# GMC-DRL/MetaBox

Measured on AMD Instinct MI355X. Metric: env-steps/sec (instances x gens/s), RLEPSO bbob-easy d=10, higher is better.
Workload: dtype f64

## Files before the change

### metabox_amd/csrc/mbx_device.hpp

```cpp
#pragma once
#include <type_traits>
#include <hip/hip_runtime.h>
#include <stdint.h>

#include "../../include/mbx.h"
#include "../../include/mbx_layout.h"
#include "mbx_math.hpp"

namespace mbx {

#ifdef MBX_NOINLINE_MATH
#define MBX_MATH __device__ __noinline__
#else
#define MBX_MATH __device__ __forceinline__
#endif
#ifdef MBX_LIBM_MATH
MBX_MATH double m_pow(double a, double b) { return pow(a, b); }
MBX_MATH double m_sin(double a) { return sin(a); }
MBX_MATH double m_cos(double a) { return cos(a); }
MBX_MATH double m_exp(double a) { return exp(a); }
MBX_MATH double m_log(double a) { return log(a); }
#else
MBX_MATH double m_pow(double a, double b) { return fm::pow_fast(a, b); }
MBX_MATH double m_sin(double a) { return fm::sincos_fast<false>(a); }
MBX_MATH double m_cos(double a) { return fm::sincos_fast<true>(a); }
MBX_MATH double m_exp(double a) { return fm::exp_fast(a); }
MBX_MATH double m_log(double a) { return fm::log_fast(a); }
#endif


constexpr int kThreads = 256;
#define MBX_NT ((int)blockDim.x)
#define MBX_NW ((int)blockDim.x >> 6)
constexpr double kTwoPi = 6.283185307179586;

struct DevProblem {
    int32_t func_id, kind, dim, n_peaks, noise_kind;
    int32_t n_close;
    double bias, lb, ub, pen_coef, s[4], noise_a, noise_b, optimum;
    const double *dshift, *m1, *m2, *v0, *v1, *v2, *py, *pc, *pw;
    const double* pyr;
    const double* plogw;
};

typedef const DevProblem __attribute__((address_space(4))) ConstProblem;

struct FastDiv {
    uint32_t m, one; int D;
    __device__ __forceinline__ explicit FastDiv(int D_) : m(0xFFFFFFFFu / (uint32_t)D_ + 1u), one(D_ == 1 ? 0xFFFFFFFFu : 0u), D(D_) {}
    __device__ __forceinline__ int div(int e) const { return (int)(__umulhi((uint32_t)e, m) + ((uint32_t)e & one)); }
    __device__ __forceinline__ int mod(int e) const { return e - div(e) * D; }
};

struct U4 { uint32_t x, y, z, w; };

__device__ __forceinline__ U4 philox4x32_10(uint32_t c0, uint32_t c1, uint32_t c2, uint32_t c3, uint32_t k0, uint32_t k1)
{
#ifndef MBX_PHILOX_ROUNDS
#define MBX_PHILOX_ROUNDS 10
#endif
#pragma unroll
    for (int r = 0; r < MBX_PHILOX_ROUNDS; ++r) {
        const uint64_t p0 = (uint64_t)MBX_PHILOX_M0 * c0, p1 = (uint64_t)MBX_PHILOX_M1 * c2;
        const uint32_t hi0 = (uint32_t)(p0 >> 32), lo0 = (uint32_t)p0;
        const uint32_t hi1 = (uint32_t)(p1 >> 32), lo1 = (uint32_t)p1;
#ifdef MBX_PHILOX_XOR2
        const uint32_t n0 = hi1 ^ c1 ^ k0, n2 = hi0 ^ c3 ^ k1;
#else
        const uint32_t n0 = __builtin_amdgcn_bitop3_b32(hi1, c1, k0, 0x96), n2 = __builtin_amdgcn_bitop3_b32(hi0, c3, k1, 0x96);
#endif
        c0 = n0; c1 = lo1; c2 = n2; c3 = lo0;
        k0 += MBX_PHILOX_W0; k1 += MBX_PHILOX_W1;
    }
    return U4{c0, c1, c2, c3};
}

__device__ __forceinline__ double u53(uint32_t a, uint32_t b)
{
    return ((double)(a >> 5) * 67108864.0 + (double)(b >> 6)) * (1.0 / 9007199254740992.0);
}

__device__ __forceinline__ double u32d(uint32_t a) { return (double)a * 2.3283064365386963e-10; }

struct Rng {
    uint32_t k0, k1, gen, episode;
    bool uniform_fresh = false;
    __device__ __forceinline__ U4 draw(uint32_t idx, uint32_t site) const
    {
#ifdef MBX_ABLATE_RNG
        return U4{idx * 2654435761u, site + 0x9E3779B9u * idx, gen ^ (idx << 7), episode + idx};
#else
        uint32_t a = k0, b = k1;
        if (uniform_fresh) {
            a = (uint32_t)__builtin_amdgcn_readfirstlane((int)a); b = (uint32_t)__builtin_amdgcn_readfirstlane((int)b);
            asm volatile("" : "+s"(a), "+s"(b));
        }
        return philox4x32_10(idx, site, gen, episode, a, b);
#endif
    }
};

__device__ __forceinline__ void box_muller(double ua, double ub, double& n0, double& n1)
{
    const double r = sqrt(-2.0 * m_log(1.0 - ua));
    const double t = kTwoPi * ub;
    n0 = r * m_cos(t);
    n1 = r * m_sin(t);
}

__device__ __forceinline__ void philox_noise(const Rng& rng, uint32_t row, uint32_t siteA, uint32_t siteB, int noise_kind,
                                             double& a, double& b, double& c)
{
    a = b = c = 0.0;
    if (noise_kind == MBX_NOISE_NONE) return;
    U4 w = rng.draw(row, siteA);
    const double ua = u53(w.x, w.y), ub = u53(w.z, w.w);
    if (noise_kind == MBX_NOISE_GAUSS) {
        a = sqrt(-2.0 * m_log(1.0 - ua)) * m_cos(kTwoPi * ub);
    } else if (noise_kind == MBX_NOISE_UNIFORM) {
        a = ua; b = ub;
    } else {
        a = ua;
        w = rng.draw(row, siteB);
        box_muller(u53(w.x, w.y), u53(w.z, w.w), b, c);
    }
}

template <class PT>
__device__ __forceinline__ double apply_noise(const PT& P, double ftrue, double a, double b, double c)
{
    if (P.noise_kind == MBX_NOISE_NONE) return ftrue;
    const double fu = ftrue - P.optimum;
    double fn;
    if (P.noise_kind == MBX_NOISE_GAUSS) {
        fn = fu * m_exp(P.noise_a * a);
    } else if (P.noise_kind == MBX_NOISE_UNIFORM) {
        fn = fu * m_pow(a, P.noise_b) * fmax(1., m_pow(1e9 / (fu + 1e-99), P.noise_a * (0.49 + 1. / P.dim) * b));
    } else {
        fn = fu + P.noise_a * fmax(0., 1e3 + (a < P.noise_b ? 1. : 0.) * b / (fabs(c) + 1e-199));
    }
    return fu >= 1e-8 ? fn + P.optimum + 1.01 * 1e-8 : ftrue;
}

__device__ __forceinline__ int opaque_tid()
{
    int t = (int)threadIdx.x;
    asm volatile("" : "+v"(t));
    return t;
}

__device__ __forceinline__ void wave_argmin(double& v, int& i)
{
#pragma unroll
    for (int off = 32; off >= 1; off >>= 1) {
        const double ov = __shfl_xor(v, off, 64);
        const int oi = __shfl_xor(i, off, 64);
        if (ov < v || (ov == v && oi < i)) { v = ov; i = oi; }
    }
}

__device__ __forceinline__ void block_argmin(const double* a, int n, double* red, double& vmin, int& imin)
{
    const int tid = opaque_tid();
    if (tid < 64) {
        double v = INFINITY; int idx = 0x7fffffff;
        for (int j = tid; j < n; j += 64) {
            const double x = a[j];
            if (x < v) { v = x; idx = j; }
        }
        wave_argmin(v, idx);
        if (idx >= n) { idx = 0; v = a[0]; }
        if (tid == 0) { red[0] = v; red[1] = (double)idx; }
    }
    __syncthreads();
    vmin = red[0]; imin = (int)red[1];
    __syncthreads();
}


__device__ __forceinline__ double div_by_tenth(double L)
{
    const double q = L * 10.0;
    return __builtin_fma(__builtin_fma(-0.1, q, L), 10.0, q);
}

__device__ __forceinline__ double osc1(double x)
{
    if (x == 0.) return x;
    const bool pos = x > 0.;
    const double y = div_by_tenth(m_log(fabs(x)));
    const double c1 = pos ? 1.0 : 0.55, c2 = pos ? 0.79 : 0.31;
    const double r = m_exp(0.1 * (y + 0.49 * (m_sin(c1 * y) + m_sin(c2 * y))));
    return pos ? r : -r;
}

#if defined(MBX_NOINLINE_MATH) && !defined(MBX_LIBM_MATH)
__device__ __noinline__ double osc1_composite(double x)
{
    if (x == 0.) return x;
    const bool pos = x > 0.;
    const double y = div_by_tenth(fm::log_fast(fabs(x)));
    const double c1 = pos ? 1.0 : 0.55, c2 = pos ? 0.79 : 0.31;
    const double r = fm::exp_fast(0.1 * (y + 0.49 * (fm::sincos_fast<false>(c1 * y) + fm::sincos_fast<false>(c2 * y))));
    return pos ? r : -r;
}
__device__ __noinline__ double schaffers_composite(double s)
{
    const double w = fm::sincos_fast<false>(50 * fm::pow_fast(s, 0.2));
    return sqrt(s) * (w * w + 1);
}
#else
__device__ __forceinline__ double osc1_composite(double x) { return osc1(x); }
__device__ __forceinline__ double schaffers_composite(double s) { return sqrt(s) * (m_pow(m_sin(50 * m_pow(s, 0.2)), 2) + 1); }
#endif
#ifndef MBX_COMPOSITE_DC
#define MBX_COMPOSITE_DC 10
#endif
template <bool CMP> __device__ __forceinline__ double osc_t(double x) { if constexpr (CMP) return osc1_composite(x); else return osc1(x); }

__device__ __forceinline__ double asy1(double x, double beta_lin)
{
    return x > 0. ? m_pow(x, 1. + beta_lin * sqrt(x)) : x;
}

__device__ __forceinline__ double pen_row(const double* x, int D, double ub)
{
    double s = 0.;
    for (int d = 0; d < D; ++d) {
        const double t = fmax(0., fabs(x[d]) - ub);
        s += t * t;
    }
    return s;
}

__host__ __device__ inline long long eval_t_doubles(int n, int D)
{
    long long t = (long long)n * D;
    if (t < 17ll * D) t = 17ll * D;
    if (t < 8ll * n) t = 8ll * n;
    return (t + 1) & ~1ll;
}

struct EvalLds {
    const double* X;
// ... 843 lines not shown
```

### metabox_amd/csrc/mbx_rlepso.hpp

```cpp
#pragma once
#include "mbx_device.hpp"

namespace mbx {

struct BatchParams {
    const DevProblem* problems;
    const int32_t* problem_idx;
    const uint64_t* seeds;
    double* state;
    int64_t state_stride;
    const double* tape;
    int64_t tape_stride;
    const int32_t* order;
    const double* pci;
    int32_t NP, D, max_fes, log_interval, n_logpoint, early_stop, n_group, B;
    int64_t sc_off;
    unsigned long long* clk;
};

template <class PT>
__device__ __forceinline__ bool log_and_terminate(const BatchParams& bp, const PT& P, double fes, double gbest, int& log_index,
                                                  int& cost_len, double* __restrict__ cost)
{
    if (fes >= (double)log_index * bp.log_interval) { log_index += 1; cost[cost_len++] = gbest; }
// ... 67 lines not shown
    L.DSH = p; p += align2(D);
    L.V0 = p; p += align2(D);
    L.V1 = p; p += align2(D);
    L.V2 = p; p += align2(D);
    L.PBC = p; p += P;
    L.NC = p; p += P;
    L.PNI = p; p += P;
    L.CMUT = p; p += P;
    L.GB = p; p += align2(D);
    L.RED = p; p += 16;
    L.IMPR = (int*)p; p += align2((P + 1) / 2);
    L.MASK = (int*)p; p += align2((P + 1) / 2);
    L.RANK = (int*)p;
    return L;
}

__device__ __forceinline__ void rl_commit(const RlLds& L, int NP, int D, bool stagnation, double& gbest, int& gbest_idx,
                                          double* __restrict__ gPB, double* __restrict__ gCC)
{
    const int tid = threadIdx.x;
    for (int i = tid; i < NP; i += MBX_NT) {
        const double nc = L.NC[i];
        if (stagnation) L.PNI[i] = nc < gCC[i] ? 0. : L.PNI[i] + 1;
        const int impr = nc < L.PBC[i];
        if (impr) L.PBC[i] = nc;
        L.IMPR[i] = impr;
        gCC[i] = nc;
    }
    double cbv; int cb;
    block_argmin(L.NC, NP, L.RED, cbv, cb);
    const bool better = cbv < gbest;
    if (better) { gbest = cbv; gbest_idx = cb; }
    const int NE = NP * D;
    const FastDiv fd(D);
    for (int e = tid; e < NE; e += MBX_NT) {
        const int i = fd.div(e);
        if (L.IMPR[i]) gPB[e] = L.X[e];
    }
    if (better && tid < D) L.GB[tid] = L.X[cb * D + tid];
    __syncthreads();
}

struct MoveCtx {
    const RlLds& L; const double* pci; const double* tape; const Rng& rng; double* gPos; double* gVel;
    const int* ORDER; const int* NLESS; const int* RANK; int NP, D, G; double lb, ub, vmax; const FastDiv& fg;
};

struct GaussMlp {
    const float* w;
    int32_t in_dim, h1, h2, out_dim;
    float min_sigma, max_sigma;
    int32_t variant;
};

__host__ __device__ inline int gauss_mlp_net_floats(int in, int h1, int h2, int A) { return in * h1 + h1 + h1 * h2 + h2 + h2 * A + A; }

__device__ __forceinline__ void gauss_head(const GaussMlp& net, float am, float as, float& mu, float& sigma)
{
    mu = (tanhf(am) + 1.f) / 2.f;
    if (net.variant == MBX_POLICY_RLPSO) sigma = fminf(fmaxf((tanhf(as) + 1.f) / 2.f, net.min_sigma), net.max_sigma);
    else sigma = (tanhf(as) + 1.f) / 2.f * (net.max_sigma - net.min_sigma) + net.min_sigma;
}

__device__ __forceinline__ float sample_action(const Rng& rng, int j, float mu, float sigma, int variant)
{
    const U4 w = rng.draw((uint32_t)j, MBX_SITE_POLICY);
    const float u1 = (float)((w.x >> 8) + 1u) * 5.9604644775390625e-8f;
    const float u2 = (float)(w.y >> 8) * 5.9604644775390625e-8f;
    const float r = __builtin_sqrtf(-1.3862943611198906f * __builtin_amdgcn_logf(u1));
    const float a = mu + sigma * (r * __builtin_amdgcn_cosf(u2));
    if (variant == MBX_POLICY_RLPSO) return fabsf(a - 0.5f) >= 0.5f ? (a + 3.f * sigma - mu) * ((1.f / 6.f) * sigma) : a;
    return fminf(fmaxf(a, 0.f), 1.f);
}

#ifdef MBX_PHASE_TIMING
__device__ unsigned long long g_phase_cycles[8192 * 16];
#define MBX_PHASE_BEGIN unsigned long long ph_t = clock64();
#define MBX_PHASE(k) do { if (threadIdx.x == 0) { const unsigned long long t_ = clock64(); g_phase_cycles[(blockIdx.x & 8191) * 16 + (k)] += t_ - ph_t; ph_t = t_; } } while (0)
#else
#define MBX_PHASE_BEGIN
#define MBX_PHASE(k)
#endif

#ifndef MBX_RL_WAVES
#define MBX_RL_WAVES __attribute__((amdgpu_waves_per_eu(THREADS == 256 ? 5 : 4)))
#endif
#ifndef MBX_FDR_UNROLL
#define MBX_FDR_UNROLL 4
#endif
#ifndef MBX_FDR_OWN_AT
#define MBX_FDR_OWN_AT 64
#endif

__device__ __forceinline__ void fdr_take(double lhs, double rhs, double& ab, double& bb, int& kb, double a, double b, int k)
{
#ifdef MBX_FDR_BRANCH
    if (__builtin_amdgcn_ballot_w64(lhs < rhs) == 0ull) return;
#endif
#ifdef MBX_FDR_SELECT
    if (lhs < rhs) { ab = a; bb = b; kb = k; }
#else
    unsigned long long saved;
    asm("s_mov_b64 %[sv], exec\n\t"
                 "v_cmpx_lt_f64_e32 %[l], %[r]\n\t"
                 "v_mov_b64 %[ab], %[a]\n\t"
                 "v_mov_b64 %[bb], %[b]\n\t"
                 "v_mov_b32 %[kb], %[k]\n\t"
                 "s_mov_b64 exec, %[sv]"
                 : [ab] "+v"(ab), [bb] "+v"(bb), [kb] "+v"(kb), [sv] "=&s"(saved)
                 : [l] "v"(lhs), [r] "v"(rhs), [a] "v"(a), [b] "v"(b), [k] "s"(k)
                 : "vcc");
#endif
}

__device__ __forceinline__ void fdr_take_neg(double dif, double& ab, double& bb, int& kb, double a, double b, int k)
{
    unsigned long long saved;
    asm("s_mov_b64 %[sv], exec\n\t"
        "v_cmpx_gt_f64_e32 0, %[d]\n\t"
        "v_mov_b64 %[ab], %[a]\n\t"
        "v_mov_b64 %[bb], %[b]\n\t"
        "v_mov_b32 %[kb], %[k]\n\t"
        "s_mov_b64 exec, %[sv]"
        : [ab] "+v"(ab), [bb] "+v"(bb), [kb] "+v"(kb), [sv] "=&s"(saved)
        : [d] "v"(dif), [a] "v"(a), [b] "v"(b), [k] "s"(k)
        : "vcc");
}
__device__ __forceinline__ void fdr_take_neg2(double dif0, double dif1, double& ab0, double& bb0, int& kb0, double& ab1, double& bb1, int& kb1,
                                              double a, double b0, double b1, int k)
{
    unsigned long long saved;
    asm("s_mov_b64 %[sv], exec\n\t"
        "v_cmpx_gt_f64_e32 0, %[d0]\n\t"
        "v_mov_b64 %[ab0], %[a]\n\t"
        "v_mov_b64 %[bb0], %[b0]\n\t"
        "v_mov_b32 %[kb0], %[k]\n\t"
        "s_mov_b64 exec, %[sv]\n\t"
        "v_cmpx_gt_f64_e32 0, %[d1]\n\t"
        "v_mov_b64 %[ab1], %[a]\n\t"
        "v_mov_b64 %[bb1], %[b1]\n\t"
        "v_mov_b32 %[kb1], %[k]\n\t"
        "s_mov_b64 exec, %[sv]"
        : [ab0] "+v"(ab0), [bb0] "+v"(bb0), [kb0] "+v"(kb0), [ab1] "+v"(ab1), [bb1] "+v"(bb1), [kb1] "+v"(kb1), [sv] "=&s"(saved)
        : [d0] "v"(dif0), [d1] "v"(dif1), [a] "v"(a), [b0] "v"(b0), [b1] "v"(b1), [k] "s"(k)
        : "vcc");
}
__device__ __forceinline__ float f64_hi_as_f32(double v) { return __int_as_float(__double2hiint(v)); }
__device__ __forceinline__ float fdr_min3_abs(float m, float x, float y)
{
    float r;
    asm("v_min3_f32 %[r], %[m], |%[x]|, |%[y]|" : [r] "=v"(r) : [m] "v"(m), [x] "v"(x), [y] "v"(y));
    return r;
}
__device__ __forceinline__ void rl_mark_copies(const RlLds& L, int NP, int D, int r)
{
    if (r > 0 && r < NP && L.NC[r] == L.NC[r - 1]) {
        bool same = true;
        for (int d = 0; d < D && same; ++d) same = L.PB[r * D + d] == L.PB[(r - 1) * D + d];
        if (same) L.NCS[r] = 1e300;
    }
}

__device__ __forceinline__ int fdr_settle(const RlLds& L, const int* __restrict__ ORDER, int D, int rk, int d, int nless, int kw, unsigned long long* cnt = nullptr)
{
    const int lane = threadIdx.x & 63;
    const double fi = L.NC[rk];
    const double pp = L.PB[rk * D + d];
    const double aw = L.NC[kw] - fi, bw = fabs(L.PB[kw * D + d] - pp) + 1e-5;
    int first_copy = 0x7fffffff;
    bool others = false;
    for (int k0 = 0; k0 < nless; k0 += 64) {
        const int k = k0 + lane;
        bool band = false, copy = false;
        if (k < nless && k != kw) {
            const double a = L.NC[k] - fi, b = fabs(L.PB[k * D + d] - pp) + 1e-5, pr = aw * b;
            band = __builtin_fma(a, bw, -pr) <= pr * -0x1p-49;
            copy = band && a == aw && b == bw;
        }
        const unsigned long long mc = __builtin_amdgcn_ballot_w64(copy), mo = __builtin_amdgcn_ballot_w64(band && !copy);
        if (mc != 0ull && first_copy == 0x7fffffff) first_copy = k0 + (int)__builtin_ctzll(mc);
        others = others || mo != 0ull;
    }
    int kbest = kw < first_copy ? kw : first_copy;
#ifdef MBX_FDR_COUNT
    if (cnt && lane == 0) atomicAdd(cnt + (others ? 5 : first_copy != 0x7fffffff ? 4 : 6), 1ull);
#endif
    if (others) {
        double qb = aw / bw;
        int ib = ORDER[kbest];
        for (int k0 = 0; k0 < nless; k0 += 64) {
            const int k = k0 + lane;
            bool cont = false;
            double qk = 0.;
            int ik = 0;
            if (k < nless && k != kw) {
                const double a = L.NC[k] - fi, b = fabs(L.PB[k * D + d] - pp) + 1e-5, pr = aw * b;
                cont = __builtin_fma(a, bw, -pr) <= pr * -0x1p-49 && !(a == aw && b == bw);
                if (cont) { qk = a / b; ik = ORDER[k]; }
            }
            unsigned long long m = __builtin_amdgcn_ballot_w64(cont);
            while (m != 0ull) {
                const int l = (int)__builtin_ctzll(m);
                m &= m - 1ull;
                const double ql = __hiloint2double(__builtin_amdgcn_readlane(__double2hiint(qk), l), __builtin_amdgcn_readlane(__double2loint(qk), l));
                const int il = __builtin_amdgcn_readlane(ik, l);
                if (ql < qb || (ql == qb && il < ib)) { qb = ql; ib = il; kbest = k0 + l; }
            }
        }
    }
    return kbest;
}

template <int W, int UN = MBX_FDR_UNROLL, bool TIE = true>
__device__ __forceinline__ bool fdr_exact(const RlLds& L, int D, int rk, int d0, int nless, int kb[W], double range = 0.)
{
#pragma unroll
    for (int q = 0; q < W; ++q) kb[q] = nless;
    if (nless <= 0) return false;
    const double fi = L.NC[rk];
    double pp[W], ab[W], bb[W];
    const double a0 = L.NC[0] - fi;
#pragma unroll
    for (int q = 0; q < W; ++q) { pp[q] = L.PB[rk * D + d0 + q]; kb[q] = 0; ab[q] = a0; bb[q] = fabs(L.PB[d0 + q] - pp[q]) + 1e-5; }
    const double* col = L.PB + d0;
    if constexpr (TIE) {
    float tiem = __int_as_float(0x7f000000);
    auto step = [&](double au, const double (&x)[W], int k) {
        double b[W], difv[W];
#pragma unroll
        for (int q = 0; q < W; ++q) b[q] = fabs(x[q] - pp[q]) + 1e-5;
#pragma unroll
        for (int q = 0; q < W; ++q) difv[q] = ab[q] * b[q];
#pragma unroll
        for (int q = 0; q < W; ++q) difv[q] = __builtin_fma(au, bb[q], -difv[q]);
        if constexpr (W == 2) fdr_take_neg2(difv[0], difv[1], ab[0], bb[0], kb[0], ab[1], bb[1], kb[1], au, b[0], b[1], k);
        else {
#pragma unroll
            for (int q = 0; q < W; ++q) fdr_take_neg(difv[q], ab[q], bb[q], kb[q], au, b[q], k);
        }
        tiem = fdr_min3_abs(tiem, f64_hi_as_f32(difv[0]), f64_hi_as_f32(difv[W - 1]));
    };
    int k = 1;
    for (; k + UN <= nless; k += UN) {
        double a[UN], x[UN][W];
#pragma unroll
        for (int u = 0; u < UN; ++u) {
            a[u] = L.NCS[k + u];
#pragma unroll
            for (int q = 0; q < W; ++q) x[u][q] = col[(k + u) * D + q];
        }
#pragma unroll
        for (int u = 0; u < UN; ++u) step(a[u] - fi, x[u], k + u);
    }
    for (; k < nless; ++k) {
        double x[W];
#pragma unroll
        for (int q = 0; q < W; ++q) x[q] = col[k * D + q];
        step(L.NCS[k] - fi, x, k);
    }
    const double thr = fabs(a0) * range * 0x1p-49;
    return !(tiem > f64_hi_as_f32(thr) * 1.0000005f);
    } else {
    int k = 1;
    for (; k + UN <= nless; k += UN) {
        double a[UN], x[UN][W];
#pragma unroll
        for (int u = 0; u < UN; ++u) {
            a[u] = L.NCS[k + u];
#pragma unroll
            for (int q = 0; q < W; ++q) x[u][q] = col[(k + u) * D + q];
        }
#pragma unroll
        for (int u = 0; u < UN; ++u) {
            const double au = a[u] - fi;
#pragma unroll
            for (int q = 0; q < W; ++q) {
                const double b = fabs(x[u][q] - pp[q]) + 1e-5;
                fdr_take(au * bb[q], ab[q] * b, ab[q], bb[q], kb[q], au, b, k + u);
            }
        }
    }
    for (; k < nless; ++k) {
        const double a = L.NCS[k] - fi;
#pragma unroll
        for (int q = 0; q < W; ++q) {
            const double b = fabs(col[k * D + q] - pp[q]) + 1e-5;
            fdr_take(a * bb[q], ab[q] * b, ab[q], bb[q], kb[q], a, b, k);
        }
    }
    return false;
    }
}

template <int W>
__device__ __noinline__ void fdr_settle_own(const double* __restrict__ NC, const double* __restrict__ PB, const int* __restrict__ ORDER, int D, int rk, int d0, int nless, int* kb)
{
    const double fi = NC[rk];
    double pp[W], aw[W], bw[W];
    int kw[W], first_copy[W];
    bool others[W];
#pragma unroll
    for (int q = 0; q < W; ++q) {
        kw[q] = kb[q];
        pp[q] = PB[rk * D + d0 + q];
        aw[q] = NC[kw[q]] - fi;
        bw[q] = fabs(PB[kw[q] * D + d0 + q] - pp[q]) + 1e-5;
        first_copy[q] = 0x7fffffff; others[q] = false;
    }
    for (int k = 0; k < nless; ++k) {
        const double a = NC[k] - fi;
#pragma unroll
        for (int q = 0; q < W; ++q) {
            const double b = fabs(PB[k * D + d0 + q] - pp[q]) + 1e-5, pr = aw[q] * b;
            if (__builtin_fma(a, bw[q], -pr) <= pr * -0x1p-49 && k != kw[q]) {
                if (a == aw[q] && b == bw[q]) { if (first_copy[q] == 0x7fffffff) first_copy[q] = k; }
                else others[q] = true;
            }
        }
    }
#pragma unroll
    for (int q = 0; q < W; ++q) {
        kb[q] = kw[q] < first_copy[q] ? kw[q] : first_copy[q];
        if (others[q]) {
            double qb = aw[q] / bw[q];
            int ib = ORDER[kb[q]];
            for (int k = 0; k < nless; ++k) {
                const double a = NC[k] - fi, b = fabs(PB[k * D + d0 + q] - pp[q]) + 1e-5, pr = aw[q] * b;
                if (__builtin_fma(a, bw[q], -pr) <= pr * -0x1p-49 && k != kw[q] && !(a == aw[q] && b == bw[q])) {
                    const double qk = a / b;
                    const int ik = ORDER[k];
                    if (qk < qb || (qk == qb && ik < ib)) { qb = qk; ib = ik; kb[q] = k; }
                }
            }
        }
    }
}

template <int W, int UN, bool TIE, int THREADS>
__device__ __forceinline__ void fdr_pass(const RlLds& L, const int* ORDER, const int* NLESS, int NP, int D, int tid, double range, unsigned long long* cnt = nullptr)
{
    const int DW = D / W, NI = NP * DW;
    const FastDiv fw(DW);
    uint32_t mine = 0;
    for (int base = 0, pass = 0; base < NI; base += THREADS, ++pass) {
        const int lim = base + THREADS < NI ? base + THREADS : NI;
        const int ps = (pass & 1) ? lim - 1 - tid : base + tid;
        if (ps >= base && ps < lim) {
            const int rk = fw.div(ps), d0 = W * (ps - rk * DW);
            int kb[W];
            const bool tie = fdr_exact<W, UN, TIE>(L, D, rk, d0, NLESS[ORDER[rk]], kb, range);
#pragma unroll
            for (int q = 0; q < W; ++q) L.KB[rk * D + d0 + q] = (uint8_t)kb[q];
#ifdef MBX_FDR_COUNT
            if (cnt) { atomicAdd(cnt + 3, 1ull); if (tie) atomicAdd(cnt + 2, 1ull); }
#endif
            if (TIE && tie) { L.FL[atomicAdd(L.FLN, 1)] = (uint16_t)ps; mine |= 1u << (pass & 31); }
        }
    }
    __syncthreads();
    if constexpr (TIE) {
        const int n = *L.FLN;
        if (n > 0 && (n <= MBX_FDR_OWN_AT || NI > 32 * THREADS)) {
            for (int c = tid >> 6; c < W * n; c += THREADS / 64) {
                const int ps = L.FL[c / W], rk = fw.div(ps), d = W * (ps - rk * DW) + c % W;
                const int kbest = fdr_settle(L, ORDER, D, rk, d, NLESS[ORDER[rk]], L.KB[rk * D + d], cnt);
                if ((tid & 63) == 0) L.KB[rk * D + d] = (uint8_t)kbest;
            }
            __syncthreads();
        } else if (n > 0) {
            for (int base = 0, pass = 0; mine != 0u; base += THREADS, ++pass, mine >>= 1) {
                if (!(mine & 1u)) continue;
// ... 241 lines not shown
        if (RANK[i] - rank > 1) {
            equal_costs = 1;
            for (int j = 0; j < i; ++j) rank += L.PBC[j] == fi;
        }
        RANK[i] = rank;
        ORDER[rank] = i; L.NC[rank] = fi; L.NCS[rank] = fi;
    }
    equal_costs = __syncthreads_or(equal_costs);
    MBX_PHASE(1);
    for (int e = tid; e < NE; e += MBX_NT) { const int i = fd.div(e), d = e - i * D; L.PB[RANK[i] * D + d] = gPB[e]; }
    __syncthreads();
    if (equal_costs) {
        for (int r = tid; r < NP; r += MBX_NT) rl_mark_copies(L, NP, D, r);
        __syncthreads();
    }
    MBX_PHASE(2);

#ifndef MBX_ABLATE_FDR
    if ((D & 1) == 0) fdr_pass<2, MBX_FDR_UNROLL, TIE, THREADS>(L, ORDER, NLESS, NP, D, tid, ub - lb + 1e-5);
    else fdr_pass<1, MBX_FDR_UNROLL, TIE, THREADS>(L, ORDER, NLESS, NP, D, tid, ub - lb + 1e-5);
#else
    for (int e = tid; e < NE; e += MBX_NT) L.KB[e] = 0;
    __syncthreads();
#endif

    const MoveCtx mc{L, bp.pci, tape, rng, gPos, gVel, ORDER, NLESS, RANK, NP, D, G, lb, ub, vmax, fg};
    if ((D & 1) == 0) {
        const int HD = D >> 1, NI = NP * HD;
        const FastDiv fh(HD);
        for (int it = tid; it < NI; it += MBX_NT) {
            const int i = fh.div(it);
            const double2 c2 = *(const double2*)(gPos + 2 * it), v2 = *(const double2*)(gVel + 2 * it);
            double cur[2] = {c2.x, c2.y}, vel[2] = {v2.x, v2.y};
            rl_move<2>(mc, i, 2 * (it - i * HD), cur, vel);
        }
    } else {
        for (int e = tid; e < NE; e += MBX_NT) {
            const int i = fd.div(e);
            double cur[1] = {gPos[e]}, vel[1] = {gVel[e]};
            rl_move<1>(mc, i, e - i * D, cur, vel);
        }
    }
    __syncthreads();
    MBX_PHASE(3);

    population_costs<eval_dc(DC), eval_md(DC)>(P, L.eval(), NP, rng, tape ? tape + MBX_RLEPSO_TAPE_NOISE0(NP, D) : nullptr, MBX_SITE_NOISE0_A, MBX_SITE_NOISE0_B);
    MBX_PHASE(4);
    fes += NP;
    rl_commit(L, NP, D, true, gbest, gbest_idx, S + MBX_RLEPSO_ST_PBPOS(NP, D), S + MBX_RLEPSO_ST_CCOST(NP, D));
    MBX_PHASE(5);

    int mine = 0;
    for (int i = tid; i < NP; i += MBX_NT) {
        double u;
        if (tape) u = tape[MBX_RLEPSO_TAPE_REINIT(NP, D) + i];
        else { const U4 w = rng.draw((uint32_t)i, MBX_SITE_REINIT); u = u53(w.x, w.y); }
        const int m = u < L.CMUT[i] * 0.01 * L.PNI[i];
        L.MASK[i] = m;
        mine += m;
    }
    const int n_reinit = __syncthreads_count(mine);
    MBX_PHASE(6);
    if (n_reinit > 0) {
        for (int e = tid; e < NE; e += MBX_NT) {
            const int i = fd.div(e);
            if (L.MASK[i]) {
                double up, uv;
                if (tape) { up = tape[MBX_RLEPSO_TAPE_REPOS(NP, D) + e]; uv = tape[MBX_RLEPSO_TAPE_REVEL(NP, D) + e]; }
                else { const U4 w = rng.draw((uint32_t)e, MBX_SITE_ELEM_R); up = u53(w.x, w.y); uv = u53(w.z, w.w); }
                const double x = lb + (ub - lb) * up;
                L.X[e] = x;
                gPos[e] = x;
                gVel[e] = -vmax + (vmax - (-vmax)) * uv;
            }
        }
        __syncthreads();
        population_costs<eval_dc(DC), eval_md(DC)>(P, L.eval(), NP, rng, tape ? tape + MBX_RLEPSO_TAPE_NOISE1(NP, D) : nullptr, MBX_SITE_NOISE1_A, MBX_SITE_NOISE1_B);
        fes += n_reinit;
        rl_commit(L, NP, D, false, gbest, gbest_idx, S + MBX_RLEPSO_ST_PBPOS(NP, D), S + MBX_RLEPSO_ST_CCOST(NP, D));
    }

    MBX_PHASE(7);
    for (int i = tid; i < NP; i += MBX_NT) {
        S[MBX_RLEPSO_ST_PBEST(NP, D) + i] = L.PBC[i];
        S[MBX_RLEPSO_ST_PNI(NP, D) + i] = L.PNI[i];
    }
    if (gbest < pre_gbest && tid < D) S[MBX_RLEPSO_ST_GBPOS(NP, D) + tid] = L.GB[tid];

    if (tid == 0) {
        int log_index = (int)sc[MBX_SC_LOG_INDEX], cost_len = (int)sc[MBX_SC_COST_LEN];
        double* cost = sc + MBX_NSCALAR;
        const bool done = log_and_terminate(bp, P, fes, gbest, log_index, cost_len, cost);
        const double reward = gbest < pre_gbest ? 1. : -1.;
        sc[MBX_SC_GBEST] = gbest; sc[MBX_SC_FES] = fes; sc[MBX_SC_LOG_INDEX] = log_index; sc[MBX_SC_COST_LEN] = cost_len;
        sc[MBX_SC_DONE] = done ? 1. : 0.; sc[MBX_SC_RETURN] += reward; sc[MBX_SC_GEN] = gen;
        sc[MBX_SC_GBEST_IDX] = gbest_idx; sc[MBX_SC_REINIT] = n_reinit > 0 ? 1. : 0.;
        if (state_out) state_out[b] = fes / bp.max_fes;
        if (reward_out) reward_out[b] = reward;
        if (done_out) done_out[b] = done ? 1 : 0;
    }
    MBX_PHASE(8);
}

struct RunOut {
    float* traj_actions;
    double* traj_state;
    double* traj_reward;
    uint8_t* traj_done;
    double* state_out;
    double* reward_out;
    uint8_t* done_out;
};

#ifndef MBX_RUN_WAVES
#define MBX_RUN_WAVES MBX_RL_WAVES
#endif
template <int THREADS, int NPC, int DC, int GC, int KIND, int NOISE, bool TIE, class ARGS>
__device__ __forceinline__ void rl_run_body(ARGS ar)
{
    const int n_gens = ar().n_gens;
    static_assert(NPC > 0 && DC > 0 && GC > 0 && (DC & 1) == 0 && NPC <= THREADS, "k_rlepso_run: compile-time geometry, even D, NP <= THREADS");
    constexpr int NP = NPC, D = DC, G = GC, HD = D / 2, NI = NP * HD, IT = (NI + THREADS - 1) / THREADS, A = 7 * G;
    extern __shared__ __attribute__((aligned(16))) double smem[];
    const int b = ar().bp.order[blockIdx.x], tid0 = threadIdx.x, tid = tid0;
    double* S = ar().bp.state + (int64_t)b * ar().bp.state_stride;
    double* sc = S + MBX_RLEPSO_ST_SCALARS(NP, D);
    const int64_t B = ar().bp.B;

    if (sc[MBX_SC_DONE] != 0.) {
        const double st = sc[MBX_SC_FES] / ar().bp.max_fes;
        for (int g = tid; g < n_gens; g += THREADS) {
            if (ar().out.traj_state) ar().out.traj_state[g * B + b] = st;
            if (ar().out.traj_reward) ar().out.traj_reward[g * B + b] = 0.;
            if (ar().out.traj_done) ar().out.traj_done[g * B + b] = 1;
        }
        if (tid == 0) {
            if (ar().out.state_out) ar().out.state_out[b] = st;
            if (ar().out.reward_out) ar().out.reward_out[b] = 0.;
            if (ar().out.done_out) ar().out.done_out[b] = 1;
        }
        return;
    }
    unsigned long long clk_c0 = 0, clk_r0 = 0;
    const bool clocked = ar().bp.clk != nullptr && tid0 == 0;
    if (clocked) { clk_c0 = __builtin_amdgcn_s_memtime(); clk_r0 = __builtin_amdgcn_s_memrealtime(); }
    ConstProblem& P = *(ConstProblem*)(ar().bp.problems + ar().bp.problem_idx[b]);
    const RlLds L = rl_carve(smem, NP, D, rl_maps_in_lds(NPC, DC));
    int gen = (int)sc[MBX_SC_GEN];
    const uint64_t seed = ar().bp.seeds[b];
    const uint32_t episode = (uint32_t)(int)sc[MBX_SC_EPISODE];
    const double lb = P.lb, ub = P.ub, vmax = 0.1 * (ub - lb);
    double gbest = sc[MBX_SC_GBEST];
    int gbest_idx = (int)sc[MBX_SC_GBEST_IDX];
    double fes = sc[MBX_SC_FES];
    int log_index = (int)sc[MBX_SC_LOG_INDEX], cost_len = (int)sc[MBX_SC_COST_LEN];
    double* cost = sc + MBX_NSCALAR;
    double ret = 0.;
    int n_reinit = 0;

    double* gPos = S + MBX_RLEPSO_ST_POS(NP, D);
    double* gVel = S + MBX_RLEPSO_ST_VEL(NP, D);
    double* gPB = S + MBX_RLEPSO_ST_PBPOS(NP, D);
    double vel[IT][2], pbp[IT][2], cc = 0.;
#pragma unroll
    for (int j = 0; j < IT; ++j) {
        const int it = tid + j * THREADS;
        vel[j][0] = vel[j][1] = pbp[j][0] = pbp[j][1] = 0.;
        if (it < NI) {
            const double2 v2 = *(const double2*)(gVel + 2 * it), p2 = *(const double2*)(gPB + 2 * it);
            vel[j][0] = v2.x; vel[j][1] = v2.y; pbp[j][0] = p2.x; pbp[j][1] = p2.y;
            *(double2*)(L.X + 2 * it) = *(const double2*)(gPos + 2 * it);
        }
    }
    if (tid < NP) {
        L.PBC[tid] = S[MBX_RLEPSO_ST_PBEST(NP, D) + tid];
        L.PNI[tid] = S[MBX_RLEPSO_ST_PNI(NP, D) + tid];
        cc = S[MBX_RLEPSO_ST_CCOST(NP, D) + tid];
    }
    if (tid < D) L.GB[tid] = S[MBX_RLEPSO_ST_GBPOS(NP, D) + tid];
    stage_problem<eval_dc(DC), eval_md(DC) == 0, ConstProblem>(P, L.eval());
    constexpr int per_group = NP / G;
    const FastDiv fg(per_group), fh(HD);
    int* ORDER = L.IMPR;
    int* NLESS = L.MASK;
    int* RANK = L.RANK;
    float* ACT = (float*)L.R1;
    int* EQC = (int*)(L.RED + 14);

    auto commit = [&](bool stagnation, int tid) {
        if (tid < NP) {
            const double nc = L.NC[tid];
            if (stagnation) L.PNI[tid] = nc < cc ? 0. : L.PNI[tid] + 1;
            const int impr = nc < L.PBC[tid];
            if (impr) L.PBC[tid] = nc;
            L.IMPR[tid] = impr;
            cc = nc;
        }
        double cbv; int cb;
        block_argmin(L.NC, NP, L.RED, cbv, cb);
        const bool better = cbv < gbest;
        if (better) { gbest = cbv; gbest_idx = cb; }
#pragma unroll
        for (int j = 0; j < IT; ++j) {
            const int it = tid + j * THREADS;
            if (it < NI && L.IMPR[fh.div(it)]) { const double2 x2 = *(const double2*)(L.X + 2 * it); pbp[j][0] = x2.x; pbp[j][1] = x2.y; }
        }
        if (better && tid < D) L.GB[tid] = L.X[cb * D + tid];
        __syncthreads();
    };

    bool done = false;
    int g = 0;
    __syncthreads();
    for (; g < n_gens && !done; ++g) {
        int tid = tid0;
        asm volatile("" : "+v"(tid));
        gen += 1;
        const Rng rng{(uint32_t)seed, (uint32_t)(seed >> 32), (uint32_t)gen, episode, true};
        const double pre_gbest = gbest;
        if (tid < A) {
            int row = (int)fes;
            row = row < ar().table_rows ? row : ar().table_rows - 1;
            const float* ms = ar().policy_table + (int64_t)row * 2 * A;
            const float a = sample_action(rng, tid, ms[tid], ms[A + tid], MBX_POLICY_RLEPSO);
            ACT[tid] = a;
            if (ar().out.traj_actions) ar().out.traj_actions[((int64_t)g * B + b) * A + tid] = a;
        }
        if (tid < NP) { NLESS[tid] = 0; ORDER[tid] = tid; }
        if (tid == 0) { *EQC = 0; *L.FLN = 0; }
        __syncthreads();
        if (tid < G) {
            const float* a = ACT + tid * G;
            const float cm = a[0] * 0.01f;
            const float wv = a[1] * 0.8f + 0.1f;
            float den = a[3] + a[4];
            den = den + a[5]; den = den + a[6]; den = den + 1e-5f;
            float scale = 1.f / den;
            scale = scale * a[2]; scale = scale * 8.f;
            double* c = L.COEF + tid * 6;
            c[0] = (double)cm; c[1] = (double)wv;
            c[2] = (double)(scale * a[3]); c[3] = (double)(scale * a[4]);
            c[4] = (double)(scale * a[5]); c[5] = (double)(scale * a[6]);
        }
        {
            constexpr int parts = THREADS / NP > 0 ? THREADS / NP : 1;
            for (int w = tid; w < parts * NP; w += THREADS) {
                const int part = w / NP, i = w - part * NP;
                const int j0 = part * NP / parts, j1 = (part + 1) * NP / parts;
                const double fi = L.PBC[i];
                int nless = 0;
#ifndef MBX_ABLATE_RANK
#pragma unroll 5
                for (int j = j0; j < j1; ++j) nless += L.PBC[j] < fi;
#else
                if (part == 0) nless = i;
#endif
                atomicAdd(&NLESS[i], nless);
            }
        }
        __syncthreads();
        if (tid < NP) {
            const int i = tid, gi = fg.div(i);
            L.CMUT[i] = gi < G ? L.COEF[gi * 6] * L.PNI[i] : 0.;
            const U4 w = rng.draw((uint32_t)i, MBX_SITE_PART);
            L.R1[i] = u53(w.x, w.y); L.R2[i] = u53(w.z, w.w);
            const int rank = NLESS[i];
            RANK[i] = rank;
            ORDER[rank] = i; L.NC[rank] = L.PBC[i]; L.NCS[rank] = L.PBC[i];
        }
        __syncthreads();
        if (tid < NP && ORDER[RANK[tid]] != tid) *EQC = 1;
        auto stage_pbest = [&](int tid) {
#pragma unroll
            for (int j = 0; j < IT; ++j) {
                const int it = tid + j * THREADS;
                if (it < NI) { const int i = fh.div(it), d0 = 2 * (it - i * HD); *(double2*)(L.PB + RANK[i] * D + d0) = double2{pbp[j][0], pbp[j][1]}; }
            }
        };
        stage_pbest(tid);
        __syncthreads();
        if (*EQC) {
            int rank = 0;
            if (tid < NP) {
                const double fi = L.PBC[tid];
                rank = NLESS[tid];
                for (int j = 0; j < tid; ++j) rank += L.PBC[j] == fi;
            }
            __syncthreads();
            if (tid < NP) { RANK[tid] = rank; ORDER[rank] = tid; L.NC[rank] = L.PBC[tid]; L.NCS[rank] = L.PBC[tid]; }
            __syncthreads();
            stage_pbest(tid);
            __syncthreads();
            rl_mark_copies(L, NP, D, tid);
            __syncthreads();
        }
#ifdef MBX_ABLATE_FDR
        for (int e = tid; e < NP * D; e += THREADS) L.KB[e] = 0;
        __syncthreads();
#else
        fdr_pass<2, (DC == 40 ? 2 : MBX_FDR_UNROLL), TIE, THREADS>(L, ORDER, NLESS, NP, D, tid, ub - lb + 1e-5, ar().bp.clk);
#endif
        {
            const MoveCtx mc{L, ar().bp.pci, nullptr, rng, nullptr, nullptr, ORDER, NLESS, RANK, NP, D, G, lb, ub, vmax, fg};
#pragma unroll
            for (int j = 0; j < IT; ++j) {
                const int it = tid + j * THREADS;
                if (it < NI) {
                    const int i = fh.div(it);
                    const double2 c2 = *(const double2*)(L.X + 2 * it);
                    double cur[2] = {c2.x, c2.y};
                    rl_move<2, true>(mc, i, 2 * (it - i * HD), cur, vel[j]);
                }
            }
        }
        __syncthreads();
        population_costs<eval_dc(DC), eval_md(DC), ConstProblem, rl_run_matvec_chunk(DC), KIND, NOISE>(P, L.eval(), NP, rng, nullptr, MBX_SITE_NOISE0_A, MBX_SITE_NOISE0_B);
        fes += NP;
        commit(true, tid);
        int mine = 0;
        if (tid < NP) {
            const U4 w = rng.draw((uint32_t)tid, MBX_SITE_REINIT);
            const double u = u53(w.x, w.y);
            mine = u < L.CMUT[tid] * 0.01 * L.PNI[tid];
            L.MASK[tid] = mine;
        }
        n_reinit = __syncthreads_count(mine);
        if (n_reinit > 0) {
#pragma unroll
            for (int j = 0; j < IT; ++j) {
                const int it = tid + j * THREADS;
                if (it < NI && L.MASK[fh.div(it)]) {
#pragma unroll
                    for (int q = 0; q < 2; ++q) {
                        const int e = 2 * it + q;
                        const U4 w = rng.draw((uint32_t)e, MBX_SITE_ELEM_R);
                        const double up = u53(w.x, w.y), uv = u53(w.z, w.w);
                        L.X[e] = lb + (ub - lb) * up;
                        vel[j][q] = -vmax + (vmax - (-vmax)) * uv;
                    }
                }
            }
            __syncthreads();
            population_costs<eval_dc(DC), eval_md(DC), ConstProblem, rl_run_matvec_chunk(DC), KIND, NOISE>(P, L.eval(), NP, rng, nullptr, MBX_SITE_NOISE1_A, MBX_SITE_NOISE1_B);
            fes += n_reinit;
            commit(false, tid);
        }
        if (fes >= (double)log_index * ar().bp.log_interval) { log_index += 1; if (tid == 0) cost[cost_len] = gbest; cost_len += 1; }
        done = fes >= ar().bp.max_fes;
        if (!isnan(P.optimum) && ar().bp.early_stop) done = done || gbest <= 1e-8;
        if (done) {
            if (cost_len >= ar().bp.n_logpoint + 1) { if (tid == 0) cost[cost_len - 1] = gbest; }
            else { if (tid == 0) cost[cost_len] = gbest; cost_len += 1; }
        }
        const double reward = gbest < pre_gbest ? 1. : -1.;
        ret += reward;
        if (tid == 0) {
            if (ar().out.traj_state) ar().out.traj_state[g * B + b] = fes / ar().bp.max_fes;
            if (ar().out.traj_reward) ar().out.traj_reward[g * B + b] = reward;
            if (ar().out.traj_done) ar().out.traj_done[g * B + b] = done ? 1 : 0;
        }
    }
#pragma unroll
    for (int j = 0; j < IT; ++j) {
        const int it = tid + j * THREADS;
        if (it < NI) {
            *(double2*)(gPos + 2 * it) = *(const double2*)(L.X + 2 * it);
            *(double2*)(gVel + 2 * it) = double2{vel[j][0], vel[j][1]};
            *(double2*)(gPB + 2 * it) = double2{pbp[j][0], pbp[j][1]};
        }
    }
    if (tid < NP) {
        S[MBX_RLEPSO_ST_PBEST(NP, D) + tid] = L.PBC[tid];
        S[MBX_RLEPSO_ST_PNI(NP, D) + tid] = L.PNI[tid];
        S[MBX_RLEPSO_ST_CCOST(NP, D) + tid] = cc;
    }
    if (tid < D) S[MBX_RLEPSO_ST_GBPOS(NP, D) + tid] = L.GB[tid];
    const double st = fes / ar().bp.max_fes;
    for (int t = g + tid; t < n_gens; t += THREADS) {
        if (ar().out.traj_state) ar().out.traj_state[t * B + b] = st;
        if (ar().out.traj_reward) ar().out.traj_reward[t * B + b] = 0.;
        if (ar().out.traj_done) ar().out.traj_done[t * B + b] = 1;
    }
    if (tid == 0) {
        sc[MBX_SC_GBEST] = gbest; sc[MBX_SC_FES] = fes; sc[MBX_SC_LOG_INDEX] = log_index; sc[MBX_SC_COST_LEN] = cost_len;
        sc[MBX_SC_DONE] = done ? 1. : 0.; sc[MBX_SC_RETURN] += ret; sc[MBX_SC_GEN] = gen;
        sc[MBX_SC_GBEST_IDX] = gbest_idx; sc[MBX_SC_REINIT] = n_reinit > 0 ? 1. : 0.;
        if (ar().out.state_out) ar().out.state_out[b] = st;
        if (ar().out.reward_out) ar().out.reward_out[b] = ret;
        if (ar().out.done_out) ar().out.done_out[b] = done ? 1 : 0;
        if (clocked) {
            atomicAdd(ar().bp.clk, (unsigned long long)__builtin_amdgcn_s_memtime() - clk_c0);
            atomicAdd(ar().bp.clk + 1, (unsigned long long)__builtin_amdgcn_s_memrealtime() - clk_r0);
        }
    }
}


struct RlRunArgs {
    BatchParams bp;
    const float* policy_table;
    int32_t table_rows, n_gens;
    RunOut out;
};

template <int THREADS, int NPC, int DC, int GC, int KIND, int NOISE, bool TIE>
__device__ __noinline__ void rl_run_body_of_kind(uint32_t karg_lo_, uint32_t karg_hi_)
{
    const uint32_t lo = (uint32_t)__builtin_amdgcn_readfirstlane((int)karg_lo_), hi = (uint32_t)__builtin_amdgcn_readfirstlane((int)karg_hi_);
    typedef const RlRunArgs __attribute__((address_space(4))) CArgs;
    auto ar = [&]() -> CArgs& {
        uintptr_t p = (uintptr_t)(((uint64_t)hi << 32) | lo);
        asm volatile("" : "+s"(p));
        return *(CArgs*)p;
    };
    rl_run_body<THREADS, NPC, DC, GC, KIND, NOISE, TIE>(ar);
}

__host__ __device__ constexpr bool rl_run_per_kind(int DC) { return DC == 10 || DC == 40; }
__host__ __device__ constexpr bool rl_run_kind_ok(int kind, int noise_kind)
{
    return noise_kind == MBX_NOISE_NONE ? (kind >= 1 && kind <= 24)
                                        : (kind == 1 || kind == 7 || kind == 8 || kind == 10 || kind == 14 || kind == 17 || kind == 19 || kind == 21);
}

template <int THREADS, int NPC, int DC, int GC, bool TIE = true>
__global__ __launch_bounds__(THREADS) MBX_RUN_WAVES void k_rlepso_run(BatchParams bp, const float* __restrict__ policy_table, int table_rows,
                                                                     int n_gens, RunOut out)
{
    if constexpr (rl_run_per_kind(DC)) {
        static_assert(sizeof(RlRunArgs) == sizeof(BatchParams) + 8 + 8 + sizeof(RunOut), "RlRunArgs mirrors the kernel's parameter list");
        const uint64_t karg = (uint64_t)(uintptr_t)__builtin_amdgcn_kernarg_segment_ptr();
        const uint32_t klo = (uint32_t)karg, khi = (uint32_t)(karg >> 32);
        const DevProblem* pr = bp.problems + bp.problem_idx[bp.order[blockIdx.x]];
        const int kind = __builtin_amdgcn_readfirstlane(pr->kind);
        const bool noisy = __builtin_amdgcn_readfirstlane(pr->noise_kind) != MBX_NOISE_NONE;
#define MBX_RL_KIND(K) case K: rl_run_body_of_kind<THREADS, NPC, DC, GC, K, 0, TIE>(klo, khi); break;
#define MBX_RL_NOISY(K) case K: rl_run_body_of_kind<THREADS, NPC, DC, GC, K, 1, TIE>(klo, khi); break;
        if (noisy) {
            switch (kind) {
            MBX_RL_NOISY(1) MBX_RL_NOISY(7) MBX_RL_NOISY(8) MBX_RL_NOISY(10) MBX_RL_NOISY(14) MBX_RL_NOISY(17) MBX_RL_NOISY(19) MBX_RL_NOISY(21)
            default: rl_run_body_of_kind<THREADS, NPC, DC, GC, 0, -1, TIE>(klo, khi);
            }
        } else {
            switch (kind) {
            MBX_RL_KIND(1) MBX_RL_KIND(2) MBX_RL_KIND(3) MBX_RL_KIND(4) MBX_RL_KIND(5) MBX_RL_KIND(6) MBX_RL_KIND(7) MBX_RL_KIND(8)
            MBX_RL_KIND(9) MBX_RL_KIND(10) MBX_RL_KIND(11) MBX_RL_KIND(12) MBX_RL_KIND(13) MBX_RL_KIND(14) MBX_RL_KIND(15) MBX_RL_KIND(16)
            MBX_RL_KIND(17) MBX_RL_KIND(18) MBX_RL_KIND(19) MBX_RL_KIND(20) MBX_RL_KIND(21) MBX_RL_KIND(22) MBX_RL_KIND(23) MBX_RL_KIND(24)
            default: rl_run_body_of_kind<THREADS, NPC, DC, GC, 0, -1, TIE>(klo, khi);
            }
        }
#undef MBX_RL_NOISY
#undef MBX_RL_KIND
    } else {
        typedef const RlRunArgs __attribute__((address_space(4))) CArgs;
        rl_run_body<THREADS, NPC, DC, GC, 0, -1, TIE>([]() -> CArgs& {
            return *(CArgs*)(uintptr_t)__builtin_amdgcn_kernarg_segment_ptr();
        });
    }
}

}
```

Baseline: 35.67 million.

## Rank pbest via wave ballots, make loop scalars integer, trim barriers

Replaces the atomic-add based per-particle rank counting with a per-wave ballot/popcount scheme that writes counts with v_writelane. The fes, log index, cost length and return become wave-uniform integers, and the reinit count uses per-wave ballots instead of __syncthreads_count. The barrier at the end of the stagnation commit is dropped, and several ablation macros are added for profiling. The aim is fewer atomics, less LDS traffic and less double-precision scalar work on the per-generation path, at the cost of relying on later barriers for correctness.

New measurement: 37.24 million, median of 6. +4.4%, better.

```diff
diff --git a/metabox_amd/csrc/mbx_device.hpp b/metabox_amd/csrc/mbx_device.hpp
--- a/metabox_amd/csrc/mbx_device.hpp
+++ b/metabox_amd/csrc/mbx_device.hpp
@@ -90,6 +90,9 @@
 #ifdef MBX_ABLATE_RNG
         return U4{idx * 2654435761u, site + 0x9E3779B9u * idx, gen ^ (idx << 7), episode + idx};
 #else
+#ifdef MBX_ABLATE_RNG_SITES
+        if (site < 32u && ((MBX_ABLATE_RNG_SITES) >> site & 1u)) return U4{idx * 2654435761u, site + 0x9E3779B9u * idx, gen ^ (idx << 7), episode + idx};
+#endif
         uint32_t a = k0, b = k1;
         if (uniform_fresh) {
             a = (uint32_t)__builtin_amdgcn_readfirstlane((int)a); b = (uint32_t)__builtin_amdgcn_readfirstlane((int)b);
diff --git a/metabox_amd/csrc/mbx_rlepso.hpp b/metabox_amd/csrc/mbx_rlepso.hpp
--- a/metabox_amd/csrc/mbx_rlepso.hpp
+++ b/metabox_amd/csrc/mbx_rlepso.hpp
@@ -243,6 +243,20 @@
     asm("v_min3_f32 %[r], %[m], |%[x]|, |%[y]|" : [r] "=v"(r) : [m] "v"(m), [x] "v"(x), [y] "v"(y));
     return r;
 }
+template <int K> struct IntC { static constexpr int value = K; };
+template <int FROM, int TO, class F>
+__device__ __forceinline__ void static_for(F&& f)
+{
+    if constexpr (FROM < TO) { f(IntC<FROM>{}); static_for<FROM + 1, TO>(f); }
+}
+template <int LANE>
+__device__ __forceinline__ int writelane_const(int val, int old)
+{
+    static_assert(LANE >= 0 && LANE < 64, "a lane of a wave");
+    asm("v_writelane_b32 %0, %1, %2" : "+v"(old) : "s"(val), "n"(LANE));
+    return old;
+}
+
 __device__ __forceinline__ void rl_mark_copies(const RlLds& L, int NP, int D, int r)
 {
     if (r > 0 && r < NP && L.NC[r] == L.NC[r - 1]) {
@@ -308,6 +322,9 @@
 #pragma unroll
     for (int q = 0; q < W; ++q) kb[q] = nless;
     if (nless <= 0) return false;
+#ifdef MBX_ABLATE_FDR_SCAN
+    nless = 1;
+#endif
     const double fi = L.NC[rk];
     double pp[W], ab[W], bb[W];
     const double a0 = L.NC[0] - fi;
@@ -855,10 +872,10 @@
     const double lb = P.lb, ub = P.ub, vmax = 0.1 * (ub - lb);
     double gbest = sc[MBX_SC_GBEST];
     int gbest_idx = (int)sc[MBX_SC_GBEST_IDX];
-    double fes = sc[MBX_SC_FES];
-    int log_index = (int)sc[MBX_SC_LOG_INDEX], cost_len = (int)sc[MBX_SC_COST_LEN];
+    int fes = __builtin_amdgcn_readfirstlane((int)sc[MBX_SC_FES]);
+    int log_index = __builtin_amdgcn_readfirstlane((int)sc[MBX_SC_LOG_INDEX]), cost_len = __builtin_amdgcn_readfirstlane((int)sc[MBX_SC_COST_LEN]);
     double* cost = sc + MBX_NSCALAR;
-    double ret = 0.;
+    int ret = 0;
     int n_reinit = 0;
 
     double* gPos = S + MBX_RLEPSO_ST_POS(NP, D);
@@ -889,6 +906,8 @@
     int* RANK = L.RANK;
     float* ACT = (float*)L.R1;
     int* EQC = (int*)(L.RED + 14);
+    int* RCNT = (int*)(L.RED + 2);
+    constexpr int PW = (NP + 63) / 64;
 
     auto commit = [&](bool stagnation, int tid) {
         if (tid < NP) {
@@ -909,7 +928,7 @@
             if (it < NI && L.IMPR[fh.div(it)]) { const double2 x2 = *(const double2*)(L.X + 2 * it); pbp[j][0] = x2.x; pbp[j][1] = x2.y; }
         }
         if (better && tid < D) L.GB[tid] = L.X[cb * D + tid];
-        __syncthreads();
+        if (!stagnation) __syncthreads();
     };
 
     bool done = false;
@@ -922,14 +941,18 @@
         const Rng rng{(uint32_t)seed, (uint32_t)(seed >> 32), (uint32_t)gen, episode, true};
         const double pre_gbest = gbest;
         if (tid < A) {
-            int row = (int)fes;
+            int row = fes;
             row = row < ar().table_rows ? row : ar().table_rows - 1;
             const float* ms = ar().policy_table + (int64_t)row * 2 * A;
+#ifndef MBX_ABLATE_POLICY
             const float a = sample_action(rng, tid, ms[tid], ms[A + tid], MBX_POLICY_RLEPSO);
+#else
+            const float a = ms[tid];
+#endif
             ACT[tid] = a;
             if (ar().out.traj_actions) ar().out.traj_actions[((int64_t)g * B + b) * A + tid] = a;
         }
-        if (tid < NP) { NLESS[tid] = 0; ORDER[tid] = tid; }
+        if (tid < NP) ORDER[tid] = tid;
         if (tid == 0) { *EQC = 0; *L.FLN = 0; }
         __syncthreads();
         if (tid < G) {
@@ -946,20 +969,23 @@
             c[4] = (double)(scale * a[5]); c[5] = (double)(scale * a[6]);
         }
         {
-            constexpr int parts = THREADS / NP > 0 ? THREADS / NP : 1;
-            for (int w = tid; w < parts * NP; w += THREADS) {
-                const int part = w / NP, i = w - part * NP;
-                const int j0 = part * NP / parts, j1 = (part + 1) * NP / parts;
-                const double fi = L.PBC[i];
-                int nless = 0;
+            static_assert(NP <= 128, "k_rlepso_run: the ranking holds two costs per lane");
+            constexpr int WAVES = THREADS / 64, PER = (NP + WAVES - 1) / WAVES;
+            const int lane = tid & 63, i0 = (tid >> 6) * PER;
+            const double flo = NP >= 64 || lane < NP ? L.PBC[NP >= 64 || lane < NP ? lane : 0] : INFINITY;
+            const double fhi = lane + 64 < NP ? L.PBC[lane + 64 < NP ? lane + 64 : 0] : INFINITY;
+            int res = 0;
 #ifndef MBX_ABLATE_RANK
-#pragma unroll 5
-                for (int j = j0; j < j1; ++j) nless += L.PBC[j] < fi;
+            static_for<0, PER>([&](auto kc) {
+                constexpr int k = decltype(kc)::value;
+                const double fi = L.PBC[PER * WAVES == NP || i0 + k < NP ? i0 + k : NP - 1];
+                const int n = __builtin_popcountll(__builtin_amdgcn_ballot_w64(flo < fi)) + __builtin_popcountll(__builtin_amdgcn_ballot_w64(fhi < fi));
+                res = writelane_const<k>(n, res);
+            });
 #else
-                if (part == 0) nless = i;
-#endif
-                atomicAdd(&NLESS[i], nless);
-            }
+            res = i0 + lane;
+#endif
+            if (lane < PER && i0 + lane < NP) NLESS[i0 + lane] = res;
         }
         __syncthreads();
         if (tid < NP) {
@@ -980,6 +1006,9 @@
                 if (it < NI) { const int i = fh.div(it), d0 = 2 * (it - i * HD); *(double2*)(L.PB + RANK[i] * D + d0) = double2{pbp[j][0], pbp[j][1]}; }
             }
         };
+#ifdef MBX_ABLATE_STAGE
+        if (g == 0)
+#endif
         stage_pbest(tid);
         __syncthreads();
         if (*EQC) {
@@ -1012,22 +1041,38 @@
                     const int i = fh.div(it);
                     const double2 c2 = *(const double2*)(L.X + 2 * it);
                     double cur[2] = {c2.x, c2.y};
+#ifndef MBX_ABLATE_MOVE
                     rl_move<2, true>(mc, i, 2 * (it - i * HD), cur, vel[j]);
+#else
+                    (void)i; (void)cur;
+#endif
                 }
             }
         }
         __syncthreads();
         population_costs<eval_dc(DC), eval_md(DC), ConstProblem, rl_run_matvec_chunk(DC), KIND, NOISE>(P, L.eval(), NP, rng, nullptr, MBX_SITE_NOISE0_A, MBX_SITE_NOISE0_B);
         fes += NP;
+#ifndef MBX_ABLATE_COMMIT
         commit(true, tid);
+#endif
         int mine = 0;
         if (tid < NP) {
+#ifndef MBX_ABLATE_REINIT_DRAW
             const U4 w = rng.draw((uint32_t)tid, MBX_SITE_REINIT);
             const double u = u53(w.x, w.y);
             mine = u < L.CMUT[tid] * 0.01 * L.PNI[tid];
+#endif
             L.MASK[tid] = mine;
         }
-        n_reinit = __syncthreads_count(mine);
+        {
+            const int cnt = __builtin_popcountll(__builtin_amdgcn_ballot_w64(mine != 0));
+            if ((tid & 63) == 0 && tid < 64 * PW) RCNT[tid >> 6] = cnt;
+            __syncthreads();
+            int n = 0;
+#pragma unroll
+            for (int w = 0; w < PW; ++w) n += RCNT[w];
+            n_reinit = __builtin_amdgcn_readfirstlane(n);
+        }
         if (n_reinit > 0) {
 #pragma unroll
             for (int j = 0; j < IT; ++j) {
@@ -1048,20 +1093,22 @@
             fes += n_reinit;
             commit(false, tid);
         }
-        if (fes >= (double)log_index * ar().bp.log_interval) { log_index += 1; if (tid == 0) cost[cost_len] = gbest; cost_len += 1; }
+#ifndef MBX_ABLATE_LOG
+        if ((int64_t)fes >= (int64_t)log_index * ar().bp.log_interval) { log_index += 1; if (tid == 0) cost[cost_len] = gbest; cost_len += 1; }
         done = fes >= ar().bp.max_fes;
-        if (!isnan(P.optimum) && ar().bp.early_stop) done = done || gbest <= 1e-8;
+        if (!isnan(P.optimum) && ar().bp.early_stop) done = done || __builtin_amdgcn_ballot_w64(gbest <= 1e-8) != 0ull;
         if (done) {
             if (cost_len >= ar().bp.n_logpoint + 1) { if (tid == 0) cost[cost_len - 1] = gbest; }
             else { if (tid == 0) cost[cost_len] = gbest; cost_len += 1; }
         }
-        const double reward = gbest < pre_gbest ? 1. : -1.;
-        ret += reward;
+        const bool improved = __builtin_amdgcn_ballot_w64(gbest < pre_gbest) != 0ull;
+        ret += improved ? 1 : -1;
         if (tid == 0) {
-            if (ar().out.traj_state) ar().out.traj_state[g * B + b] = fes / ar().bp.max_fes;
-            if (ar().out.traj_reward) ar().out.traj_reward[g * B + b] = reward;
+            if (ar().out.traj_state) ar().out.traj_state[g * B + b] = (double)fes / ar().bp.max_fes;
+            if (ar().out.traj_reward) ar().out.traj_reward[g * B + b] = improved ? 1. : -1.;
             if (ar().out.traj_done) ar().out.traj_done[g * B + b] = done ? 1 : 0;
         }
+#endif
     }
 #pragma unroll
     for (int j = 0; j < IT; ++j) {
@@ -1078,7 +1125,7 @@
         S[MBX_RLEPSO_ST_CCOST(NP, D) + tid] = cc;
     }
     if (tid < D) S[MBX_RLEPSO_ST_GBPOS(NP, D) + tid] = L.GB[tid];
-    const double st = fes / ar().bp.max_fes;
+    const double st = (double)fes / ar().bp.max_fes;
     for (int t = g + tid; t < n_gens; t += THREADS) {
         if (ar().out.traj_state) ar().out.traj_state[t * B + b] = st;
         if (ar().out.traj_reward) ar().out.traj_reward[t * B + b] = 0.;
```
